# bigmat18/cuda-mesh-voxelization

Measured on AMD Instinct MI355X. Metric: Mvoxels/s (voxelize+JFA) at N=512, bunny 1.35M tris, higher is better.
Workload: dtype f32

## Files before the change

cuda_mesh_voxelization_amd/csrc/jfa_dense.hip:

```cpp
#include "jfa_common.h"

namespace vp {
namespace {

template <class ID> constexpr bool final_mask_global() { return ID::kTab > 512; }
constexpr int kStoreAux = 2;
template <int PM>
__device__ __forceinline__ float from_partner(float v)
{
    constexpr int ctrl = PM == 1 ? 0xB1 : PM == 2 ? 0x4E : PM == 4 ? 0x141 : 0x128;
    return __builtin_bit_cast(float, __builtin_amdgcn_update_dpp(0, __builtin_bit_cast(int, v), ctrl, 0xf, 0xf, true));
}
template <class ID, int RY, int NT, bool FINAL>
constexpr int dense_waves()
{
    return std::is_same<ID, IdC>::value ? 4 : RY > 4 ? 4 : (FINAL && !final_mask_global<ID>()) ? (ID::kTab == 512 ? 5 : 4) : (ID::kTab == 512 || NT == 512) ? 6 : 4;
}
template <class ID, int RY, int CH, int NT, bool FINAL, int PM, int CLOSED = 0, bool FULL = false, bool CYC = false>
__global__ void __launch_bounds__(NT, (dense_waves<ID, RY, NT, FINAL>()))
jfa_pass_dense(Frame f, uint32_t kArg, uint32_t ka, const char* __restrict__ in, const char* __restrict__ inB, char* __restrict__ out, char* __restrict__ outB,
               const char* __restrict__ none_row, const uint32_t* __restrict__ words, float fill, float* __restrict__ sdf,
               uint32_t tilesY, uint32_t tiles, uint32_t splitTiles, uint32_t cyc)
{
    static_assert(!CYC || !FINAL, "the last pass (k = 1) is never a multiple of the rank count");
    using T = typename ID::T;
    constexpr bool CPT = std::is_same<ID, IdC>::value;
    constexpr uint32_t IDB = 4u;
    constexpr int TAB = ID::kTab;
    constexpr int PXT = CPT ? TAB : TAB + 1;
    constexpr int TABZ = CPT ? IdC::kTabZ : TAB;
    constexpr int HY = (CLOSED & 1) ? 0 : 1;
    constexpr bool CZ = (CLOSED & 2) != 0;
    constexpr int NR = RY + 2 * HY;
    static_assert(!CLOSED || !FINAL, "closed tiles: id passes");
    constexpr int NC = PM ? 2 : 3;
    constexpr int NI = NR * NC;
    constexpr int CHT = CPT ? 1 : CH;
    using B = typename std::conditional<FINAL, float, double>::type;
    __shared__ float PX[PXT];
    __shared__ float TY[RY][TAB];
    __shared__ float TZ[CHT][TABZ];
    __shared__ uint32_t RB[CPT ? (CH + 2) * NR : 1];
    constexpr bool GM = final_mask_global<ID>();
    __shared__ uint32_t WM[(FINAL && !GM) ? RY * CH * (TAB / 32) : 1];

    const int N = (int)f.n;
    const uint32_t k = FINAL ? 1u : kArg;
    const int K = (int)k;
    const int zsh = CYC ? (int)(cyc & 31u) : 0, zoff = CYC ? (int)(cyc >> 8) : 0;
    const int KZ = CYC ? K >> zsh : K, NZ = CYC ? N >> zsh : N;
    auto zglobal = [&](int l) { return CYC ? zoff + (l << zsh) : l; };
    const int nzl = (int)(f.z1 - f.z0);
    const uint32_t tid = threadIdx.x;
    const int nresY = min(K, N);
    const bool rev = ((31 - __builtin_clz(k)) & 1) != 0;
    uint32_t lin = blockIdx.x;
    const uint32_t total = tiles;
    uint32_t xpart = 0, xparts = 1;
    if (lin >= total - splitTiles) {
        const uint32_t u = lin - (total - splitTiles);
        lin = total - splitTiles + (u >> 1); xpart = u & 1u; xparts = 2;
    }
    {
        const uint32_t whole8 = (total - splitTiles) & ~7u;
        if (K < 8 && lin < whole8) lin = (lin & 7u) * (whole8 >> 3) + (lin >> 3);
    }
    if (rev) lin = total - 1u - lin;
    const int nres = min(KZ, nzl);
    uint32_t bx, by, bxq, bxr, byq, byr;
    udivmod(lin, tilesY, by, bx); udivmod(bx, (uint32_t)nresY, bxq, bxr);
    const int ybase = (int)bxr + (int)bxq * RY * K;
    udivmod(by, (uint32_t)nres, byq, byr);
    const int lbase = (int)byr + (int)byq * CH * KZ;
    if (ybase >= N || lbase >= nzl) return;
    const int zbase = lbase + (int)f.z0;
    const int KA = (int)ka;
    float py[RY], pz[CH];
#pragma unroll
    for (int j = 0; j < RY; ++j) py[j] = axis_pos(f.oy, ybase + j * K, f.vs);
#pragma unroll
    for (int j = 0; j < CH; ++j) pz[j] = axis_pos(f.oz, zglobal(zbase + j * KZ), f.vs);
    for (uint32_t i = tid; i < (uint32_t)PXT; i += NT) PX[i] = i < (uint32_t)N ? axis_pos(f.ox, i, f.vs) : INFINITY;
    for (uint32_t i = tid; i < (uint32_t)TAB; i += NT) {
        if (i < (uint32_t)N) {
            const uint32_t si = scr(i);
            const float sy = axis_pos(f.oy, i, f.vs), sz = axis_pos(f.oz, i, f.vs);
#pragma unroll
            for (int j = 0; j < RY; ++j) { const float d = sy - py[j]; TY[j][si] = d * d; }
            if (CPT) TZ[0][si] = sz;
            else {
#pragma unroll
                for (int j = 0; j < CHT; ++j) { const float d = sz - pz[j]; TZ[j][si] = d * d; }
            }
        } else {
#pragma unroll
            for (int j = 0; j < RY; ++j) TY[j][i] = 0.0f;
#pragma unroll
            for (int j = 0; j < CHT; ++j) TZ[j][i] = 0.0f;
        }
    }
    if constexpr (TABZ > TAB)
        for (uint32_t i = (uint32_t)TAB + tid; i < (uint32_t)TABZ; i += NT) TZ[0][i] = INFINITY;
    if (CPT) {
        for (uint32_t i = tid; i < (uint32_t)((CH + 2) * NR); i += NT) {
            const int pj = (int)(i / NR) - 1, zg = zbase + pj * KZ, yy = ybase + ((int)(i % NR) - HY) * K;
            const bool ok = zg >= (int)f.z0 - KZ && zg < (int)f.z1 + KZ && zg >= 0 && zg < NZ && yy >= 0 && yy < N;
            RB[i] = ok ? (uint32_t)((lbase + pj * KA) * N + yy) : 0u;
        }
    }
    if (FINAL && !GM) {
        for (uint32_t i = tid; i < (uint32_t)(RY * CH) * f.w; i += NT) {
            uint32_t ou, c;
            udivmod(i, f.w, ou, c);
            const int o = (int)ou, a = o / CH, j = o % CH;
            const int oy = ybase + a * K, oz = zbase + j * K;
            WM[o * (TAB / 32) + (int)c] = (oy < N && oz < (int)f.z1) ? words[(uint32_t)((oz - (int)f.z0) * N + oy) * f.w + c] : 0u;
        }
    }
    __syncthreads();

    const char* tx = reinterpret_cast<const char*>(PX);
    const char* ty = reinterpret_cast<const char*>(TY);
    const char* tz = reinterpret_cast<const char*>(TZ);
    const uint32_t rowBytes = (uint32_t)N * IDB;
    const size_t planeBytes = (size_t)N * rowBytes;
    const char* noneB = none_row + (size_t)TAB * 4u;
    int yout = 1, nout = 1;
    if constexpr (FULL) { yout = RY; nout = CH; }
    else {
#pragma unroll
        for (int j = 1; j < RY; ++j) yout += (ybase + j * K < N) ? 1 : 0;
#pragma unroll
        for (int j = 1; j < CH; ++j) nout += (zbase + j * KZ < (int)f.z1) ? 1 : 0;
    }
    const uint32_t kb = k * IDB;

    const int zbase0 = zbase, lbase0 = lbase, ybase0 = ybase;
    const uint32_t xiters = ((uint32_t)N + NT - 1) / NT, xper = (xiters + xparts - 1) / xparts * NT;
    const uint32_t xbeg = xpart * xper, xend = min((uint32_t)N, xbeg + xper);
    for (uint32_t xb = xbeg; xb < xend; xb += NT) {
        uint32_t x = xb + tid;
        bool upper = false;
        if constexpr (PM != 0) {
            uint32_t pl;
            if (PM == 1) { upper = tid & 1u; pl = tid >> 1; }
            else if (PM == 2) { upper = (tid >> 1) & 1u; pl = ((tid >> 2) << 1) | (tid & 1u); }
            else if (PM == 4) { const uint32_t l8 = tid & 7u; upper = l8 >> 2; pl = ((tid >> 3) << 2) | (upper ? 7u - l8 : l8); }
            else { upper = (tid >> 3) & 1u; pl = ((tid >> 4) << 3) | (tid & 7u); }
            const uint32_t pr = (xb >> 1) + pl;
            x = (((pr & ~(k - 1u)) << 1) | (pr & (k - 1u))) + (upper ? k : 0u);
        } else if (x >= xend) break;
        const int zbase = (int)opaque_uniform((size_t)(uint32_t)zbase0), lbase = (int)opaque_uniform((size_t)(uint32_t)lbase0);
        const int ybase = (int)opaque_uniform((size_t)(uint32_t)ybase0);
        const int plo = zbase - KZ >= 0 ? -1 : 0;
        const char* gbase = in + (ptrdiff_t)(lbase + plo * KA) * (ptrdiff_t)planeBytes;
        uint32_t ro[NR];
        bool yv[NR];
#pragma unroll
        for (int rr = 0; rr < NR; ++rr) {
            const int ny = ybase + (rr - HY) * K;
            yv[rr] = ny >= 0 && ny < N && max(rr - HY - 1, 0) < yout;
            ro[rr] = (uint32_t)(yv[rr] ? ny : 0) * rowBytes;
        }
        const float px = PX[x];
        const bool hasM = x >= k, hasP = x + k < (uint32_t)N;
        const uint32_t xo = x * IDB, xmo = hasM ? xo - kb : xo, xpo = hasP ? xo + kb : xo;
        const uint32_t xpart = upper ? xo - kb : xo + kb, xout = upper ? xpo : xmo;
        const uint32_t xoB = xo >> 2, xmoB = xmo >> 2, xpoB = xpo >> 2, xoutB = xout >> 2;

        struct Plane { const char* base; const char* baseB; bool ok; };
        auto plane_of = [&](int P, bool needed) {
            Plane pl;
            const int zg = zbase + P * KZ;
            pl.ok = needed && zg >= 0 && zg < NZ;
            const ptrdiff_t wp = pl.ok ? (ptrdiff_t)(lbase + P * KA) : 0;
            pl.base = opaque_uniform(in + wp * (ptrdiff_t)planeBytes);
            pl.baseB = CPT ? opaque_uniform(inB + wp * (ptrdiff_t)((size_t)N * N)) : nullptr;
            return pl;
        };
        auto load_row = [&](const Plane& pl, int rr, T (&w)[NI]) {
            const bool ok = pl.ok && yv[rr];
            const __amdgpu_buffer_rsrc_t b = row_resource(ok ? pl.base + ro[rr] : none_row, rowBytes);
            if constexpr (CPT) {
                const __amdgpu_buffer_rsrc_t bb = row_resource(ok ? pl.baseB + (ro[rr] >> 2) : noneB, (uint32_t)N);
                if constexpr (PM != 0) {
                    uint32_t w0, w1;
                    row_load(w0, b, xo); row_load(w1, b, xout);
                    w[rr * 2 + 0] = make_uint2(w0, row_load_u8(bb, xoB));
                    w[rr * 2 + 1] = make_uint2(w1, row_load_u8(bb, xoutB));
                } else {
                    uint32_t w0, w1, w2;
                    row_load(w0, b, xmo); row_load(w1, b, xo); row_load(w2, b, xpo);
                    w[rr * 3 + 0] = make_uint2(w0, row_load_u8(bb, xmoB));
                    w[rr * 3 + 1] = make_uint2(w1, row_load_u8(bb, xoB));
                    w[rr * 3 + 2] = make_uint2(w2, row_load_u8(bb, xpoB));
                }
            } else if constexpr (PM != 0) {
                row_load(w[rr * 2 + 0], b, xo);
                row_load(w[rr * 2 + 1], b, xout);
            } else {
                row_load(w[rr * 3 + 0], b, xmo);
                row_load(w[rr * 3 + 1], b, xo);
                row_load(w[rr * 3 + 2], b, xpo);
            }
        };

        B best[RY][CH];

        struct Dec { float sx; float dy2[RY]; float dz2[CH]; uint32_t zt; };
        auto lookup = [&](int P, int rr, T id, Dec& d) {
            const int alo = max(rr - HY - 1, 0), ahi = min(rr - HY + 1, RY - 1), olo = max(P - 1, 0), ohi = min(P + 1, CH - 1);
            d.sx = lds_f32(tx + ID::xoff(id));
            if constexpr (CPT) d.zt = ID::zt2(id); else d.zt = 0u;
            const uint32_t yo = ID::yoff(id), zo = ID::zoff(id);
#pragma unroll
            for (int a = alo; a <= ahi; ++a) d.dy2[a] = lds_f32(ty + a * (TAB * 4) + yo);
            if constexpr (CPT) {
                const float sz = lds_f32(tz + zo);
#pragma unroll
                for (int o = olo; o <= ohi; ++o) { const float dzv = sz - pz[o]; d.dz2[o] = dzv * dzv; }
            } else {
#pragma unroll
                for (int o = olo; o <= ohi; ++o) d.dz2[o] = lds_f32(tz + o * (TAB * 4) + zo);
            }
        };
        float hold[3][3];
        auto steps_col = [&](int P, int rr, int c, bool ownCol, uint32_t coloff, const Dec& d, uint32_t prank, auto dppv) {
            constexpr bool DPPV = decltype(dppv)::value;
            auto val = [&](float v) { if constexpr (DPPV) return from_partner<PM ? PM : 1>(v); else return v; };
            auto valu = [&](uint32_t v) { if constexpr (DPPV) return __float_as_uint(from_partner<PM ? PM : 1>(__uint_as_float(v))); else return v; };
            const int alo = max(rr - HY - 1, 0), ahi = min(rr - HY + 1, RY - 1), olo = max(P - 1, 0), ohi = min(P + 1, CH - 1);
            const float dxv = val(d.sx) - px;
            const float dx2 = dxv * dxv;
            u32x2 cand;
            if (!FINAL) {
                if constexpr (CPT) cand.x = (uint32_t)(((P + 1) * NR + rr + 1) << 14) + 1u + coloff + valu(d.zt);
                else cand.x = prank + ro[rr] + coloff;
            }
#pragma unroll
            for (int a = alo; a <= ahi; ++a) {
                const float pre = val(d.dy2[a]) + dx2;
                const bool ownRow = (rr == a + HY) && ownCol;
#pragma unroll
                for (int o = olo; o <= ohi; ++o) {
                    const float dd = val(d.dz2[o]) + pre;
                    if constexpr (FINAL) {
                        if (c == 0) hold[a - alo][o - olo] = dd;
                        else if (c == 1) best[a][o] = min3_f32(best[a][o], hold[a - alo][o - olo], dd);
                        else best[a][o] = min_f32(best[a][o], dd);
                    } else {
                        u32x2 cd = cand;
                        if (ownRow && o == P) cd.x = CPT ? d.zt : 0u;
                        cd.y = __float_as_uint(dd);
                        best[a][o] = min_f64(best[a][o], __builtin_bit_cast(double, cd));
                    }
                }
            }
        };
        auto steps = [&](int P, int rr, int c, const Dec& d, uint32_t prank) {
            if constexpr (PM != 0) {
                if (c == 0) {
                    steps_col(P, rr, 0, true, xo, d, prank, std::false_type{});
                    steps_col(P, rr, 1, false, xpart, d, prank, std::true_type{});
                } else {
                    steps_col(P, rr, 2, false, xout, d, prank, std::false_type{});
                }
            } else {
                steps_col(P, rr, c, c == 1, c == 0 ? xmo : c == 1 ? xo : xpo, d, prank, std::false_type{});
            }
        };
        constexpr bool PIPE = ID::kTab == 512 || (FINAL && !CPT);
        auto scatter = [&](int P, T (&w)[NI]) {
            const uint32_t prank = CPT ? 0u : (uint32_t)((P - plo) * KA) * (uint32_t)planeBytes + 1u;
            const int olo = max(P - 1, 0), ohi = min(P + 1, CH - 1);
            Plane next{nullptr, nullptr, false};
            const bool roll = P + 1 <= CH - (CZ ? 1 : 0);
            if (roll) next = plane_of(P + 1, P + 1 <= nout);
            if constexpr (PIPE) {
                constexpr int DEPTH = (FINAL && ID::kTab == 1024) ? 2 : 1;
                Dec d[DEPTH + 1];
#pragma unroll
                for (int j = 0; j < DEPTH && j < NI; ++j) lookup(P, j / NC, w[j], d[j]);
#pragma unroll
                for (int j = 0; j < NI; ++j) {
                    const int rr = j / NC, c = j % NC;
                    if (j + DEPTH < NI) lookup(P, (j + DEPTH) / NC, w[j + DEPTH], d[(j + DEPTH) % (DEPTH + 1)]);
                    __builtin_amdgcn_sched_barrier(0);
                    steps(P, rr, c, d[j % (DEPTH + 1)], prank);
                    if (c == NC - 1) {
                        const int alo = max(rr - HY - 1, 0), ahi = min(rr - HY + 1, RY - 1);
#pragma unroll
                        for (int a = alo; a <= ahi; ++a)
#pragma unroll
                            for (int o = olo; o <= ohi; ++o) pin(best[a][o]);
                        if (roll) load_row(next, rr, w);
                    }
                    __builtin_amdgcn_sched_barrier(0);
                }
                return;
            }
#pragma unroll
            for (int rr = 0; rr < NR; ++rr) {
                const int alo = max(rr - HY - 1, 0), ahi = min(rr - HY + 1, RY - 1);
#pragma unroll
                for (int c = 0; c < NC; ++c) {
                    Dec d;
                    lookup(P, rr, w[rr * NC + c], d);
                    steps(P, rr, c, d, prank);
                }
#pragma unroll
                for (int a = alo; a <= ahi; ++a)
#pragma unroll
                    for (int o = olo; o <= ohi; ++o) pin(best[a][o]);
                if (roll) load_row(next, rr, w);
            }
        };

        T w[NI];
        T pend[RY];
        {
            const Plane first = plane_of(CZ ? 0 : -1, true);
#pragma unroll
            for (int rr = 0; rr < NR; ++rr) load_row(first, rr, w);
        }
#pragma clang loop unroll(full)
        for (int P = -1; P <= CH; ++P) {
            if (P + 1 < CH) {
#pragma unroll
                for (int a = 0; a < RY; ++a) {
                    if constexpr (FINAL) best[a][P + 1] = INFINITY;
                    else best[a][P + 1] = __builtin_bit_cast(double, (u32x2){0xFFFFFFFFu, 0x7F800000u});
                }
            }
            uint32_t mw[RY] = {};
            if constexpr (FINAL && GM) {
                if (P >= 1 && P - 1 < nout) {
                    const char* wpl = opaque_uniform(reinterpret_cast<const char*>(words) + ((size_t)(lbase + (P - 1) * K) * N + ybase) * (size_t)(f.w * 4u));
                    const __amdgpu_buffer_rsrc_t wr = row_resource(wpl, (uint32_t)(RY * K) * f.w * 4u);
#pragma unroll
                    for (int a = 0; a < RY; ++a) {
                        if (a >= yout) continue;
                        mw[a] = (uint32_t)__builtin_amdgcn_raw_buffer_load_b32(wr, (int)((x >> 5) << 2), (int)((uint32_t)(a * K) * f.w * 4u), 0);
                    }
                }
            }
            if (!(CZ && (P == -1 || P == CH))) scatter(P, w);
            if constexpr (FINAL) {
                if (P >= 1 && P - 1 < nout) {
                    const char* spl = opaque_uniform(reinterpret_cast<const char*>(sdf) + ((size_t)(lbase + (P - 1) * K) * N + ybase) * (size_t)rowBytes);
                    const __amdgpu_buffer_rsrc_t sr = row_resource(spl, (uint32_t)((RY - 1) * K + 1) * rowBytes);
#pragma unroll
                    for (int a = 0; a < RY; ++a) {
                        if (a >= yout) continue;
                        const bool set = ((GM ? mw[a] : WM[(a * CH + (P - 1)) * (TAB / 32) + (x >> 5)]) >> (x & 31)) & 1u;
                        __builtin_amdgcn_raw_buffer_store_b32(__float_as_uint(set ? best[a][P - 1] : copysignf(best[a][P - 1], fill)), sr, (int)xo,
                                                              (int)((uint32_t)(a * K) * rowBytes), kStoreAux);
                    }
                }
            } else {
                if (P >= 2 && P - 2 < nout) {
                    const char* orow = opaque_uniform(out + ((size_t)(lbase + (P - 2) * KA) * N + ybase) * rowBytes);
                    const char* orowB = CPT ? opaque_uniform(outB + ((size_t)(lbase + (P - 2) * KA) * N + ybase) * (size_t)N) : nullptr;
#pragma unroll
                    for (int a = 0; a < RY; ++a) {
                        if (a >= yout) continue;
                        if constexpr (CPT) {
                            row_store<kStoreAux>(pend[a].x, row_resource(orow + (size_t)(a * K) * rowBytes, rowBytes), xo);
                            row_store_u8<kStoreAux>(pend[a].y, row_resource(orowB + (size_t)(a * K) * N, (uint32_t)N), xoB);
                        } else {
                            row_store<kStoreAux>(pend[a], row_resource(orow + (size_t)(a * K) * rowBytes, rowBytes), xo);
                        }
                    }
                }
                if (P >= 1 && P - 1 < nout) {
                    const uint32_t orank = (uint32_t)((P - 1 - plo) * KA) * (uint32_t)planeBytes;
#pragma unroll
                    for (int a = 0; a < RY; ++a) {
                        if (a >= yout) continue;
                        const uint32_t lo = __builtin_bit_cast(u32x2, best[a][P - 1]).x;
                        if constexpr (CPT) {
                            const uint32_t zt = lo & 2u;
                            const uint32_t r = lo < 4u ? (uint32_t)((P * NR + a + HY + 1) << 14) + xo : lo - 1u - zt;
                            const ptrdiff_t row = (ptrdiff_t)(int)RB[(r >> 14) - 1u];
                            const uint32_t none1 = __builtin_bit_cast(u32x2, best[a][P - 1]).y == 0x7F800000u ? IdC::kNoneBit : 0u;
                            pend[a] = make_uint2(*reinterpret_cast<const uint32_t*>(in + row * (ptrdiff_t)rowBytes + (ptrdiff_t)(r & 16383u)),
                                                 zt | none1);
                        } else {
                            const uint32_t ownOff = orank + ro[a + HY] + xo;
                            const uint32_t off = lo ? lo - 1u : ownOff;
                            pend[a] = *reinterpret_cast<const T*>(gbase + off);
                        }
                    }
                }
            }
#pragma unroll
            for (int a = 0; a < RY; ++a)
#pragma unroll
                for (int o = P; o <= P + 1; ++o)
                    if (o >= 0 && o < CH) pin(best[a][o]);
        }
        if constexpr (!FINAL) {
            if (CH - 1 < nout) {
                const char* orow = opaque_uniform(out + ((size_t)(lbase + (CH - 1) * KA) * N + ybase) * rowBytes);
                const char* orowB = CPT ? opaque_uniform(outB + ((size_t)(lbase + (CH - 1) * KA) * N + ybase) * (size_t)N) : nullptr;
#pragma unroll
                for (int a = 0; a < RY; ++a) {
                    if (a >= yout) continue;
                    if constexpr (CPT) {
                        row_store<kStoreAux>(pend[a].x, row_resource(orow + (size_t)(a * K) * rowBytes, rowBytes), xo);
                        row_store_u8<kStoreAux>(pend[a].y, row_resource(orowB + (size_t)(a * K) * N, (uint32_t)N), xoB);
                    } else {
                        row_store<kStoreAux>(pend[a], row_resource(orow + (size_t)(a * K) * rowBytes, rowBytes), xo);
                    }
                }
            }
        }
    }
}

}

static uint32_t tail_split(const vp_ctx* ctx, uint32_t tiles, uint32_t wgPerCu)
{
    const uint32_t slots = (uint32_t)ctx->cus * wgPerCu;
    if (tiles >= 16u * slots) return 0;
    return std::min(tiles / 2u, slots * 4u / 3u);
}

struct DenseArgs {
    vp_ctx* ctx; Frame f; uint32_t k, ka;
    const char *in, *inB; char *out, *outB; const char* none_row;
    const uint32_t* words; float fill; float* sdf;
    uint32_t nresY, ylen, nres, zlen;
    uint32_t cyc = 0;
};
int launch_dense_id9_tile16(const DenseArgs& a, bool pairsOk);

namespace {

template <class ID, int RY, int CH, int NT, bool F, int PM, int CL = 0, bool FULL = false, bool CYC = false>
void launch_tile(const DenseArgs& a)
{
    const uint32_t ty = a.nresY * ((a.ylen + RY - 1) / RY), t = ty * a.nres * ((a.zlen + CH - 1) / CH);
    constexpr uint32_t perCu = std::is_same<ID, IdC>::value ? 2u
                             : ID::kTab == 512 ? (RY == 8 ? 4u : (F && !final_mask_global<ID>()) ? 5u : 6u)
                             : NT == 512 ? (RY == 8 ? 2u : 3u) : 4u;
    const uint32_t sp = a.f.n > (uint32_t)NT ? tail_split(a.ctx, t, perCu) : 0u;
    hipLaunchKernelGGL((jfa_pass_dense<ID, RY, CH, NT, F, PM, CL, FULL, CYC>), dim3(t + sp), dim3(NT), 0, a.ctx->stream, a.f, a.k, a.ka,
                       a.in, a.inB, a.out, a.outB, a.none_row, a.words, a.fill, a.sdf, ty, t, sp, a.cyc);
}

template <int V> using int_c = std::integral_constant<int, V>;

template <class ID, int CH, int NT, bool F, bool ALWAYS_FULL = false, bool CYC = false>
void launch_shape(const DenseArgs& a, bool pairsOk, bool wholeChains)
{
    constexpr int RY = (ID::kTab == 512 && !F && CH >= 8) ? 8 : 4;
    constexpr bool canFull = CH >= 8 && (ID::kTab != 1024 || F);
    auto go = [&](auto pm) {
        constexpr int PM = decltype(pm)::value;
        if constexpr (ALWAYS_FULL || (CYC && canFull)) launch_tile<ID, RY, CH, NT, F, PM, 0, true, CYC>(a);
        else {
            if constexpr (canFull) {
                if (wholeChains && a.ylen % RY == 0) { launch_tile<ID, RY, CH, NT, F, PM, 0, true>(a); return; }
            }
            launch_tile<ID, RY, CH, NT, F, PM, 0, false, CYC>(a);
        }
    };
    if constexpr (CH >= 8) {
        if (pairsOk && a.f.n % NT == 0) {
            if constexpr (F) { go(int_c<1>{}); return; }
            else {
                if constexpr (ID::kTab != 512) { if (a.k == 2) { go(int_c<2>{}); return; } }
                if (a.k == 4) { go(int_c<4>{}); return; }
                if (a.k >= 8) { go(int_c<8>{}); return; }
            }
        }
    }
    go(int_c<0>{});
}

template <class ID, bool FIN>
int launch_dense(vp_ctx* ctx, const Frame& f, uint32_t k, const IdWin& in, const IdWin& out, uint32_t stride,
                 const uint32_t* d_words, float fill, float* d_sdf)
{
    const uint32_t nz = f.z1 - f.z0, n = f.n;
    constexpr bool fin = FIN;
    const uint32_t nres = std::min(k, nz), zlen = (nz + k - 1) / k;
    const uint32_t nresY = std::min(k, n), ylen = (n + k - 1) / k;
    if (stride == k && nz % k == 0 && k < nz && zlen > 8 && zlen % 8 != 0) {
        const uint32_t planesA = (zlen / 8u) * 8u * k;
        Frame fa = f, fb = f;
        fa.z1 = f.z0 + planesA; fb.z0 = fa.z1;
        IdWin inB = in, outB = out;
        inB.at += planesA; outB.at += planesA;
        const size_t wordPlane = (size_t)n * f.w, sdfPlane = (size_t)n * n;
        VP_TRY((launch_dense<ID, FIN>(ctx, fa, k, in, out, stride, d_words, fill, d_sdf)));
        return launch_dense<ID, FIN>(ctx, fb, k, inB, outB, stride, d_words ? d_words + planesA * wordPlane : nullptr, fill, d_sdf ? d_sdf + planesA * sdfPlane : nullptr);
    }
    if (FIN && k != 1) return set_error(VP_ERR_INVALID, "jfa_pass_dense: the fused last pass is the pass with k = 1");
    VP_TRY(ensure_none_rows(ctx));
    DenseArgs a{ctx, f, k, stride, win_words(in, n, in.at), win_compact(n) ? win_bytes_plane(in, n, in.at) : nullptr,
                win_words(out, n, out.at), win_compact(n) ? win_bytes_plane(out, n, out.at) : nullptr,
                (const char*)(std::is_same<ID, Id9>::value ? none_row_id9(ctx) : std::is_same<ID, Id10>::value ? none_row_id10(ctx) : none_row_idc(ctx)),
                d_words, fill, d_sdf, nresY, ylen, nres, zlen};
    const bool pow2 = (n & (n - 1)) == 0;
    const bool wholeChains = zlen % 8 == 0 && nz % k == 0 && n % k == 0;
    constexpr int NTD = ID::kTab == 512 ? 256 : 512;
    constexpr int NTS = ID::kTab == 2048 ? 512 : 256;
    if constexpr (!std::is_same<ID, IdC>::value) {
        if constexpr (!fin) {
            if (pow2 && stride == k && f.z0 == 0 && f.z1 == n && n == 8u * k && n % NTD == 0) {
                launch_tile<ID, 8, 8, NTD, false, 8, 3, ID::kTab == 512>(a);
                VP_HIP(hipGetLastError());
                return 0;
            }
        }
    }
    const bool deep = zlen % 8 == 0 || (zlen > 4 && zlen < 8);
    const bool tiny = zlen <= 2;
    if constexpr (std::is_same<ID, IdC>::value) {
        if (zlen % 16 == 0 && stride == k) {
            launch_shape<ID, 16, NTD, fin>(a, pow2 && (fin || k >= 2), wholeChains);
            VP_HIP(hipGetLastError());
            return 0;
        }
    }
    if constexpr (ID::kTab == 512) {
        if (n == 512 && zlen % 16 == 0 && stride == k && wholeChains) {
            if constexpr (fin) launch_shape<ID, 16, 512, true, true>(a, pow2, true);
            else VP_TRY(launch_dense_id9_tile16(a, pow2 && k >= 2));
            VP_HIP(hipGetLastError());
            return 0;
        }
    }
    if (deep) launch_shape<ID, 8, NTD, fin>(a, pow2 && (fin || k >= 2), wholeChains);
    else if constexpr (!fin) { if (tiny) launch_shape<ID, 2, NTS, false>(a, false, false); else launch_shape<ID, 4, NTS, false>(a, false, false); }
    else launch_shape<ID, 4, NTS, true>(a, false, false);
    VP_HIP(hipGetLastError());
    return 0;
}

template <class ID>
int launch_dense_cyclic(vp_ctx* ctx, const Frame& f, uint32_t k, const IdWin& in, const IdWin& out, uint32_t ranks, uint32_t rank)
{
    const uint32_t n = f.n, zsh = (uint32_t)__builtin_ctz(ranks);
    const uint32_t nzl = n >> zsh, kz = k >> zsh;
    if ((ranks & (ranks - 1)) != 0 || rank >= ranks || n % ranks != 0 || k % ranks != 0 || n % k != 0 || n / k < 8 || ((n / k) & (n / k - 1)) != 0)
        return set_error(VP_ERR_INVALID, "jfa_pass_dense (cyclic): n = %u, k = %u, %u ranks", n, k, ranks);
    VP_TRY(ensure_none_rows(ctx));
    Frame fl = f;
    fl.z0 = 0; fl.z1 = nzl;
    const uint32_t zlen = nzl / kz, ylen = n / k;
    DenseArgs a{ctx, fl, k, kz, win_words(in, n, in.at), win_compact(n) ? win_bytes_plane(in, n, in.at) : nullptr,
                win_words(out, n, out.at), win_compact(n) ? win_bytes_plane(out, n, out.at) : nullptr,
                (const char*)(std::is_same<ID, Id9>::value ? none_row_id9(ctx) : std::is_same<ID, Id10>::value ? none_row_id10(ctx) : none_row_idc(ctx)),
                nullptr, 0.0f, nullptr, std::min(k, n), ylen, std::min(kz, nzl), zlen, zsh | (rank << 8)};
    const bool pow2 = (n & (n - 1)) == 0;
    constexpr int NTD = ID::kTab == 512 ? 256 : 512;
    if constexpr (!std::is_same<ID, IdC>::value) {
        if (pow2 && n == 8u * k && n % NTD == 0) {
            launch_tile<ID, 8, 8, NTD, false, 8, 3, ID::kTab == 512, true>(a);
            VP_HIP(hipGetLastError());
            return 0;
        }
    }
    if constexpr (std::is_same<ID, IdC>::value) {
        if (zlen % 16 == 0) {
            launch_shape<ID, 16, NTD, false, false, true>(a, pow2 && k >= 2, true);
            VP_HIP(hipGetLastError());
            return 0;
        }
    }
    launch_shape<ID, 8, NTD, false, false, true>(a, pow2 && k >= 2, true);
    VP_HIP(hipGetLastError());
    return 0;
}

}

#ifndef VP_DENSE_PART
#define VP_DENSE_PART 0
#endif
#define VP_DENSE_ENTRY(PART, NAME, ID, FIN)                                                                                                \
    int NAME(vp_ctx* ctx, const Frame& f, uint32_t k, const IdWin& in, const IdWin& out, uint32_t stride, const uint32_t* d_words, float fill, float* d_sdf) \
    { return launch_dense<ID, FIN>(ctx, f, k, in, out, stride, d_words, fill, d_sdf); }
#if VP_DENSE_PART == 0 || VP_DENSE_PART == 1
VP_DENSE_ENTRY(1, launch_dense_id9_pass, Id9, false)
#endif
#if VP_DENSE_PART == 0 || VP_DENSE_PART == 2
VP_DENSE_ENTRY(2, launch_dense_id9_last, Id9, true)
#endif
#if VP_DENSE_PART == 0 || VP_DENSE_PART == 3
VP_DENSE_ENTRY(3, launch_dense_id10_pass, Id10, false)
#endif
#if VP_DENSE_PART == 0 || VP_DENSE_PART == 4
VP_DENSE_ENTRY(4, launch_dense_id10_last, Id10, true)
#endif
#if VP_DENSE_PART == 0 || VP_DENSE_PART == 5
VP_DENSE_ENTRY(5, launch_dense_idc_pass, IdC, false)
#endif
#if VP_DENSE_PART == 0 || VP_DENSE_PART == 6
VP_DENSE_ENTRY(6, launch_dense_idc_last, IdC, true)
#endif
#if VP_DENSE_PART == 0 || VP_DENSE_PART == 7
int launch_dense_id9_tile16(const DenseArgs& a, bool pairsOk) { launch_shape<Id9, 16, 512, false, true>(a, pairsOk, true); return 0; }
#endif
#undef VP_DENSE_ENTRY
#define VP_CYCLIC_ENTRY(NAME, ID)                                                                                                        \
    int NAME(vp_ctx* ctx, const Frame& f, uint32_t k, const IdWin& in, const IdWin& out, uint32_t ranks, uint32_t rank)                 \
    { return launch_dense_cyclic<ID>(ctx, f, k, in, out, ranks, rank); }
#if VP_DENSE_PART == 0 || VP_DENSE_PART == 8
VP_CYCLIC_ENTRY(launch_cyclic_id9_pass, Id9)
#endif
#if VP_DENSE_PART == 0 || VP_DENSE_PART == 9
VP_CYCLIC_ENTRY(launch_cyclic_id10_pass, Id10)
#endif
#if VP_DENSE_PART == 0 || VP_DENSE_PART == 10
VP_CYCLIC_ENTRY(launch_cyclic_idc_pass, IdC)
#endif
#undef VP_CYCLIC_ENTRY

}
```

Measured before the change: 49430.

## Add chain-end tile variants that skip absent halo rows and planes in JFA passes

Splits the dense JFA pass body into a device function and adds ENDS-specialised launches for k=32 and k=16 at N=512. Tiles at the ends of a y or z chain are walked in mirrored direction, so the missing neighbour row or plane is always on the low side and can be dropped at compile time. The closed-tile flags are split into separate lo/hi bits. This cuts halo loads and distance evaluations for edge tiles, at the cost of more template instances, run-time branching between variants and negative-stride addressing.

```diff
diff --git a/cuda_mesh_voxelization_amd/csrc/jfa_dense.hip b/cuda_mesh_voxelization_amd/csrc/jfa_dense.hip
--- a/cuda_mesh_voxelization_amd/csrc/jfa_dense.hip
+++ b/cuda_mesh_voxelization_amd/csrc/jfa_dense.hip
@@ -11,38 +11,52 @@
     constexpr int ctrl = PM == 1 ? 0xB1 : PM == 2 ? 0x4E : PM == 4 ? 0x141 : 0x128;
     return __builtin_bit_cast(float, __builtin_amdgcn_update_dpp(0, __builtin_bit_cast(int, v), ctrl, 0xf, 0xf, true));
 }
+constexpr int kNoRowLo = 1, kNoRowHi = 2;
+constexpr int kNoPlaneLo = 4, kNoPlaneHi = 8;
+constexpr int kClosedTile = kNoRowLo | kNoRowHi | kNoPlaneLo | kNoPlaneHi;
 template <class ID, int RY, int NT, bool FINAL>
 constexpr int dense_waves()
 {
     return std::is_same<ID, IdC>::value ? 4 : RY > 4 ? 4 : (FINAL && !final_mask_global<ID>()) ? (ID::kTab == 512 ? 5 : 4) : (ID::kTab == 512 || NT == 512) ? 6 : 4;
 }
-template <class ID, int RY, int CH, int NT, bool FINAL, int PM, int CLOSED = 0, bool FULL = false, bool CYC = false>
-__global__ void __launch_bounds__(NT, (dense_waves<ID, RY, NT, FINAL>()))
-jfa_pass_dense(Frame f, uint32_t kArg, uint32_t ka, const char* __restrict__ in, const char* __restrict__ inB, char* __restrict__ out, char* __restrict__ outB,
-               const char* __restrict__ none_row, const uint32_t* __restrict__ words, float fill, float* __restrict__ sdf,
-               uint32_t tilesY, uint32_t tiles, uint32_t splitTiles, uint32_t cyc)
-{
-    static_assert(!CYC || !FINAL, "the last pass (k = 1) is never a multiple of the rank count");
+
+template <class ID, int RY, int CH, bool FINAL>
+struct DenseLds {
+    static constexpr bool CPT = std::is_same<ID, IdC>::value;
+    static constexpr int TAB = ID::kTab;
+    static constexpr int PXT = CPT ? TAB : TAB + 1;
+    static constexpr int TABZ = CPT ? IdC::kTabZ : TAB;
+    static constexpr int CHT = CPT ? 1 : CH;
+    static constexpr int RBN = CPT ? (CH + 2) * (RY + 2) : 1;
+    static constexpr int WMN = (FINAL && !final_mask_global<ID>()) ? RY * CH * (TAB / 32) : 1;
+    float (&PX)[PXT];
+    float (&TY)[RY][TAB];
+    float (&TZ)[CHT][TABZ];
+    uint32_t (&RB)[RBN];
+    uint32_t (&WM)[WMN];
+};
+
+template <class ID, int RY, int CH, int NT, bool FINAL, int PM, int CLOSED, bool FULL, bool CYC, bool MIR = false>
+__device__ __forceinline__ void
+dense_tile(const DenseLds<ID, RY, CH, FINAL>& lds, const Frame& f, uint32_t kArg, uint32_t ka, const char* __restrict__ in, const char* __restrict__ inB,
+           char* __restrict__ out, char* __restrict__ outB, const char* __restrict__ none_row, const uint32_t* __restrict__ words, float fill,
+           float* __restrict__ sdf, uint32_t cyc, uint32_t xpart, uint32_t xparts, int ybase, int lbase, bool miry, bool mirz)
+{
     using T = typename ID::T;
-    constexpr bool CPT = std::is_same<ID, IdC>::value;
+    using LDS = DenseLds<ID, RY, CH, FINAL>;
+    constexpr bool CPT = LDS::CPT;
     constexpr uint32_t IDB = 4u;
-    constexpr int TAB = ID::kTab;
-    constexpr int PXT = CPT ? TAB : TAB + 1;
-    constexpr int TABZ = CPT ? IdC::kTabZ : TAB;
-    constexpr int HY = (CLOSED & 1) ? 0 : 1;
-    constexpr bool CZ = (CLOSED & 2) != 0;
-    constexpr int NR = RY + 2 * HY;
-    static_assert(!CLOSED || !FINAL, "closed tiles: id passes");
+    constexpr int TAB = LDS::TAB, PXT = LDS::PXT, TABZ = LDS::TABZ, CHT = LDS::CHT;
+    constexpr int HYlo = (CLOSED & kNoRowLo) ? 0 : 1, HYhi = (CLOSED & kNoRowHi) ? 0 : 1;
+    constexpr bool NZlo = (CLOSED & kNoPlaneLo) != 0, NZhi = (CLOSED & kNoPlaneHi) != 0;
+    constexpr int NR = RY + HYlo + HYhi;
+    static_assert(!CLOSED || (!FINAL && !CPT), "closed tiles: id passes on 32-bit ids");
+    static_assert(!MIR || (!FINAL && !CPT && !CYC && FULL), "run-time walk directions: whole tiles of the 32-bit id passes");
     constexpr int NC = PM ? 2 : 3;
     constexpr int NI = NR * NC;
-    constexpr int CHT = CPT ? 1 : CH;
     using B = typename std::conditional<FINAL, float, double>::type;
-    __shared__ float PX[PXT];
-    __shared__ float TY[RY][TAB];
-    __shared__ float TZ[CHT][TABZ];
-    __shared__ uint32_t RB[CPT ? (CH + 2) * NR : 1];
+    auto& PX = lds.PX; auto& TY = lds.TY; auto& TZ = lds.TZ; auto& RB = lds.RB; auto& WM = lds.WM;
     constexpr bool GM = final_mask_global<ID>();
-    __shared__ uint32_t WM[(FINAL && !GM) ? RY * CH * (TAB / 32) : 1];
 
     const int N = (int)f.n;
     const uint32_t k = FINAL ? 1u : kArg;
@@ -50,36 +64,15 @@
     const int zsh = CYC ? (int)(cyc & 31u) : 0, zoff = CYC ? (int)(cyc >> 8) : 0;
     const int KZ = CYC ? K >> zsh : K, NZ = CYC ? N >> zsh : N;
     auto zglobal = [&](int l) { return CYC ? zoff + (l << zsh) : l; };
-    const int nzl = (int)(f.z1 - f.z0);
     const uint32_t tid = threadIdx.x;
-    const int nresY = min(K, N);
-    const bool rev = ((31 - __builtin_clz(k)) & 1) != 0;
-    uint32_t lin = blockIdx.x;
-    const uint32_t total = tiles;
-    uint32_t xpart = 0, xparts = 1;
-    if (lin >= total - splitTiles) {
-        const uint32_t u = lin - (total - splitTiles);
-        lin = total - splitTiles + (u >> 1); xpart = u & 1u; xparts = 2;
-    }
-    {
-        const uint32_t whole8 = (total - splitTiles) & ~7u;
-        if (K < 8 && lin < whole8) lin = (lin & 7u) * (whole8 >> 3) + (lin >> 3);
-    }
-    if (rev) lin = total - 1u - lin;
-    const int nres = min(KZ, nzl);
-    uint32_t bx, by, bxq, bxr, byq, byr;
-    udivmod(lin, tilesY, by, bx); udivmod(bx, (uint32_t)nresY, bxq, bxr);
-    const int ybase = (int)bxr + (int)bxq * RY * K;
-    udivmod(by, (uint32_t)nres, byq, byr);
-    const int lbase = (int)byr + (int)byq * CH * KZ;
-    if (ybase >= N || lbase >= nzl) return;
     const int zbase = lbase + (int)f.z0;
     const int KA = (int)ka;
+    const int SK = (MIR && miry) ? -K : K, SKZ = (MIR && mirz) ? -KZ : KZ, SKA = (MIR && mirz) ? -KA : KA;
     float py[RY], pz[CH];
 #pragma unroll
-    for (int j = 0; j < RY; ++j) py[j] = axis_pos(f.oy, ybase + j * K, f.vs);
-#pragma unroll
-    for (int j = 0; j < CH; ++j) pz[j] = axis_pos(f.oz, zglobal(zbase + j * KZ), f.vs);
+    for (int j = 0; j < RY; ++j) py[j] = axis_pos(f.oy, ybase + j * SK, f.vs);
+#pragma unroll
+    for (int j = 0; j < CH; ++j) pz[j] = axis_pos(f.oz, zglobal(zbase + j * SKZ), f.vs);
     for (uint32_t i = tid; i < (uint32_t)PXT; i += NT) PX[i] = i < (uint32_t)N ? axis_pos(f.ox, i, f.vs) : INFINITY;
     for (uint32_t i = tid; i < (uint32_t)TAB; i += NT) {
         if (i < (uint32_t)N) {
@@ -103,7 +96,7 @@
         for (uint32_t i = (uint32_t)TAB + tid; i < (uint32_t)TABZ; i += NT) TZ[0][i] = INFINITY;
     if (CPT) {
         for (uint32_t i = tid; i < (uint32_t)((CH + 2) * NR); i += NT) {
-            const int pj = (int)(i / NR) - 1, zg = zbase + pj * KZ, yy = ybase + ((int)(i % NR) - HY) * K;
+            const int pj = (int)(i / NR) - 1, zg = zbase + pj * KZ, yy = ybase + ((int)(i % NR) - HYlo) * K;
             const bool ok = zg >= (int)f.z0 - KZ && zg < (int)f.z1 + KZ && zg >= 0 && zg < NZ && yy >= 0 && yy < N;
             RB[i] = ok ? (uint32_t)((lbase + pj * KA) * N + yy) : 0u;
         }
@@ -152,14 +145,14 @@
         } else if (x >= xend) break;
         const int zbase = (int)opaque_uniform((size_t)(uint32_t)zbase0), lbase = (int)opaque_uniform((size_t)(uint32_t)lbase0);
         const int ybase = (int)opaque_uniform((size_t)(uint32_t)ybase0);
-        const int plo = zbase - KZ >= 0 ? -1 : 0;
-        const char* gbase = in + (ptrdiff_t)(lbase + plo * KA) * (ptrdiff_t)planeBytes;
+        const int plo = (MIR && mirz) ? ((!NZhi && zbase + CH * SKZ >= 0) ? CH : CH - 1) : ((!NZlo && zbase - KZ >= 0) ? -1 : 0);
+        const char* gbase = in + (ptrdiff_t)(lbase + plo * SKA) * (ptrdiff_t)planeBytes;
         uint32_t ro[NR];
         bool yv[NR];
 #pragma unroll
         for (int rr = 0; rr < NR; ++rr) {
-            const int ny = ybase + (rr - HY) * K;
-            yv[rr] = ny >= 0 && ny < N && max(rr - HY - 1, 0) < yout;
+            const int ny = ybase + (rr - HYlo) * SK;
+            yv[rr] = ny >= 0 && ny < N && max(rr - HYlo - 1, 0) < yout;
             ro[rr] = (uint32_t)(yv[rr] ? ny : 0) * rowBytes;
         }
         const float px = PX[x];
@@ -171,9 +164,9 @@
         struct Plane { const char* base; const char* baseB; bool ok; };
         auto plane_of = [&](int P, bool needed) {
             Plane pl;
-            const int zg = zbase + P * KZ;
+            const int zg = zbase + P * SKZ;
             pl.ok = needed && zg >= 0 && zg < NZ;
-            const ptrdiff_t wp = pl.ok ? (ptrdiff_t)(lbase + P * KA) : 0;
+            const ptrdiff_t wp = pl.ok ? (ptrdiff_t)(lbase + P * SKA) : 0;
             pl.base = opaque_uniform(in + wp * (ptrdiff_t)planeBytes);
             pl.baseB = CPT ? opaque_uniform(inB + wp * (ptrdiff_t)((size_t)N * N)) : nullptr;
             return pl;
@@ -209,7 +202,7 @@
 
         struct Dec { float sx; float dy2[RY]; float dz2[CH]; uint32_t zt; };
         auto lookup = [&](int P, int rr, T id, Dec& d) {
-            const int alo = max(rr - HY - 1, 0), ahi = min(rr - HY + 1, RY - 1), olo = max(P - 1, 0), ohi = min(P + 1, CH - 1);
+            const int alo = max(rr - HYlo - 1, 0), ahi = min(rr - HYlo + 1, RY - 1), olo = max(P - 1, 0), ohi = min(P + 1, CH - 1);
             d.sx = lds_f32(tx + ID::xoff(id));
             if constexpr (CPT) d.zt = ID::zt2(id); else d.zt = 0u;
             const uint32_t yo = ID::yoff(id), zo = ID::zoff(id);
@@ -229,7 +222,7 @@
             constexpr bool DPPV = decltype(dppv)::value;
             auto val = [&](float v) { if constexpr (DPPV) return from_partner<PM ? PM : 1>(v); else return v; };
             auto valu = [&](uint32_t v) { if constexpr (DPPV) return __float_as_uint(from_partner<PM ? PM : 1>(__uint_as_float(v))); else return v; };
-            const int alo = max(rr - HY - 1, 0), ahi = min(rr - HY + 1, RY - 1), olo = max(P - 1, 0), ohi = min(P + 1, CH - 1);
+            const int alo = max(rr - HYlo - 1, 0), ahi = min(rr - HYlo + 1, RY - 1), olo = max(P - 1, 0), ohi = min(P + 1, CH - 1);
             const float dxv = val(d.sx) - px;
             const float dx2 = dxv * dxv;
             u32x2 cand;
@@ -240,7 +233,7 @@
 #pragma unroll
             for (int a = alo; a <= ahi; ++a) {
                 const float pre = val(d.dy2[a]) + dx2;
-                const bool ownRow = (rr == a + HY) && ownCol;
+                const bool ownRow = (rr == a + HYlo) && ownCol;
 #pragma unroll
                 for (int o = olo; o <= ohi; ++o) {
                     const float dd = val(d.dz2[o]) + pre;
@@ -271,10 +264,10 @@
         };
         constexpr bool PIPE = ID::kTab == 512 || (FINAL && !CPT);
         auto scatter = [&](int P, T (&w)[NI]) {
-            const uint32_t prank = CPT ? 0u : (uint32_t)((P - plo) * KA) * (uint32_t)planeBytes + 1u;
+            const uint32_t prank = CPT ? 0u : (uint32_t)((P - plo) * SKA) * (uint32_t)planeBytes + 1u;
             const int olo = max(P - 1, 0), ohi = min(P + 1, CH - 1);
             Plane next{nullptr, nullptr, false};
-            const bool roll = P + 1 <= CH - (CZ ? 1 : 0);
+            const bool roll = P + 1 <= CH - (NZhi ? 1 : 0);
             if (roll) next = plane_of(P + 1, P + 1 <= nout);
             if constexpr (PIPE) {
                 constexpr int DEPTH = (FINAL && ID::kTab == 1024) ? 2 : 1;
@@ -288,7 +281,7 @@
                     __builtin_amdgcn_sched_barrier(0);
                     steps(P, rr, c, d[j % (DEPTH + 1)], prank);
                     if (c == NC - 1) {
-                        const int alo = max(rr - HY - 1, 0), ahi = min(rr - HY + 1, RY - 1);
+                        const int alo = max(rr - HYlo - 1, 0), ahi = min(rr - HYlo + 1, RY - 1);
 #pragma unroll
                         for (int a = alo; a <= ahi; ++a)
 #pragma unroll
@@ -301,7 +294,7 @@
             }
 #pragma unroll
             for (int rr = 0; rr < NR; ++rr) {
-                const int alo = max(rr - HY - 1, 0), ahi = min(rr - HY + 1, RY - 1);
+                const int alo = max(rr - HYlo - 1, 0), ahi = min(rr - HYlo + 1, RY - 1);
 #pragma unroll
                 for (int c = 0; c < NC; ++c) {
                     Dec d;
@@ -319,7 +312,7 @@
         T w[NI];
         T pend[RY];
         {
-            const Plane first = plane_of(CZ ? 0 : -1, true);
+            const Plane first = plane_of(NZlo ? 0 : -1, true);
 #pragma unroll
             for (int rr = 0; rr < NR; ++rr) load_row(first, rr, w);
         }
@@ -344,7 +337,7 @@
                     }
                 }
             }
-            if (!(CZ && (P == -1 || P == CH))) scatter(P, w);
+            if (!((NZlo && P == -1) || (NZhi && P == CH))) scatter(P, w);
             if constexpr (FINAL) {
                 if (P >= 1 && P - 1 < nout) {
                     const char* spl = opaque_uniform(reinterpret_cast<const char*>(sdf) + ((size_t)(lbase + (P - 1) * K) * N + ybase) * (size_t)rowBytes);
@@ -359,8 +352,8 @@
                 }
             } else {
                 if (P >= 2 && P - 2 < nout) {
-                    const char* orow = opaque_uniform(out + ((size_t)(lbase + (P - 2) * KA) * N + ybase) * rowBytes);
-                    const char* orowB = CPT ? opaque_uniform(outB + ((size_t)(lbase + (P - 2) * KA) * N + ybase) * (size_t)N) : nullptr;
+                    const char* orow = opaque_uniform(out + ((size_t)(lbase + (P - 2) * SKA) * N + ybase) * rowBytes);
+                    const char* orowB = CPT ? opaque_uniform(outB + ((size_t)(lbase + (P - 2) * SKA) * N + ybase) * (size_t)N) : nullptr;
 #pragma unroll
                     for (int a = 0; a < RY; ++a) {
                         if (a >= yout) continue;
@@ -368,25 +361,26 @@
                             row_store<kStoreAux>(pend[a].x, row_resource(orow + (size_t)(a * K) * rowBytes, rowBytes), xo);
                             row_store_u8<kStoreAux>(pend[a].y, row_resource(orowB + (size_t)(a * K) * N, (uint32_t)N), xoB);
                         } else {
-                            row_store<kStoreAux>(pend[a], row_resource(orow + (size_t)(a * K) * rowBytes, rowBytes), xo);
+                            if constexpr (MIR) row_store<kStoreAux>(pend[a], row_resource(orow + (ptrdiff_t)(a * SK) * (ptrdiff_t)rowBytes, rowBytes), xo);
+                            else row_store<kStoreAux>(pend[a], row_resource(orow + (size_t)(a * K) * rowBytes, rowBytes), xo);
                         }
                     }
                 }
                 if (P >= 1 && P - 1 < nout) {
-                    const uint32_t orank = (uint32_t)((P - 1 - plo) * KA) * (uint32_t)planeBytes;
+                    const uint32_t orank = (uint32_t)((P - 1 - plo) * SKA) * (uint32_t)planeBytes;
 #pragma unroll
                     for (int a = 0; a < RY; ++a) {
                         if (a >= yout) continue;
                         const uint32_t lo = __builtin_bit_cast(u32x2, best[a][P - 1]).x;
                         if constexpr (CPT) {
                             const uint32_t zt = lo & 2u;
-                            const uint32_t r = lo < 4u ? (uint32_t)((P * NR + a + HY + 1) << 14) + xo : lo - 1u - zt;
+                            const uint32_t r = lo < 4u ? (uint32_t)((P * NR + a + HYlo + 1) << 14) + xo : lo - 1u - zt;
                             const ptrdiff_t row = (ptrdiff_t)(int)RB[(r >> 14) - 1u];
                             const uint32_t none1 = __builtin_bit_cast(u32x2, best[a][P - 1]).y == 0x7F800000u ? IdC::kNoneBit : 0u;
                             pend[a] = make_uint2(*reinterpret_cast<const uint32_t*>(in + row * (ptrdiff_t)rowBytes + (ptrdiff_t)(r & 16383u)),
                                                  zt | none1);
                         } else {
-                            const uint32_t ownOff = orank + ro[a + HY] + xo;
+                            const uint32_t ownOff = orank + ro[a + HYlo] + xo;
                             const uint32_t off = lo ? lo - 1u : ownOff;
                             pend[a] = *reinterpret_cast<const T*>(gbase + off);
                         }
@@ -401,8 +395,8 @@
         }
         if constexpr (!FINAL) {
             if (CH - 1 < nout) {
-                const char* orow = opaque_uniform(out + ((size_t)(lbase + (CH - 1) * KA) * N + ybase) * rowBytes);
-                const char* orowB = CPT ? opaque_uniform(outB + ((size_t)(lbase + (CH - 1) * KA) * N + ybase) * (size_t)N) : nullptr;
+                const char* orow = opaque_uniform(out + ((size_t)(lbase + (CH - 1) * SKA) * N + ybase) * rowBytes);
+                const char* orowB = CPT ? opaque_uniform(outB + ((size_t)(lbase + (CH - 1) * SKA) * N + ybase) * (size_t)N) : nullptr;
 #pragma unroll
                 for (int a = 0; a < RY; ++a) {
                     if (a >= yout) continue;
@@ -410,10 +404,75 @@
                         row_store<kStoreAux>(pend[a].x, row_resource(orow + (size_t)(a * K) * rowBytes, rowBytes), xo);
                         row_store_u8<kStoreAux>(pend[a].y, row_resource(orowB + (size_t)(a * K) * N, (uint32_t)N), xoB);
                     } else {
-                        row_store<kStoreAux>(pend[a], row_resource(orow + (size_t)(a * K) * rowBytes, rowBytes), xo);
+                        if constexpr (MIR) row_store<kStoreAux>(pend[a], row_resource(orow + (ptrdiff_t)(a * SK) * (ptrdiff_t)rowBytes, rowBytes), xo);
+                        else row_store<kStoreAux>(pend[a], row_resource(orow + (size_t)(a * K) * rowBytes, rowBytes), xo);
                     }
                 }
             }
+        }
+    }
+}
+
+template <class ID, int RY, int CH, int NT, bool FINAL, int PM, int CLOSED = 0, bool FULL = false, bool CYC = false, int ENDS = 0>
+__global__ void __launch_bounds__(NT, (dense_waves<ID, RY, NT, FINAL>()))
+jfa_pass_dense(Frame f, uint32_t kArg, uint32_t ka, const char* __restrict__ in, const char* __restrict__ inB, char* __restrict__ out, char* __restrict__ outB,
+               const char* __restrict__ none_row, const uint32_t* __restrict__ words, float fill, float* __restrict__ sdf,
+               uint32_t tilesY, uint32_t tiles, uint32_t splitTiles, uint32_t cyc)
+{
+    static_assert(!CYC || !FINAL, "the last pass (k = 1) is never a multiple of the rank count");
+    static_assert(!ENDS || (!CLOSED && FULL && !CYC && !FINAL), "chain-end tiles: whole tiles of the id passes of a whole grid");
+    using LDS = DenseLds<ID, RY, CH, FINAL>;
+    __shared__ float PX[LDS::PXT];
+    __shared__ float TY[RY][LDS::TAB];
+    __shared__ float TZ[LDS::CHT][LDS::TABZ];
+    __shared__ uint32_t RB[LDS::RBN];
+    __shared__ uint32_t WM[LDS::WMN];
+    const LDS lds{PX, TY, TZ, RB, WM};
+
+    const int N = (int)f.n;
+    const uint32_t k = FINAL ? 1u : kArg;
+    const int K = (int)k;
+    const int KZ = CYC ? K >> (int)(cyc & 31u) : K;
+    const int nzl = (int)(f.z1 - f.z0);
+    const int nresY = min(K, N);
+    const bool rev = ((31 - __builtin_clz(k)) & 1) != 0;
+    uint32_t lin = blockIdx.x;
+    const uint32_t total = tiles;
+    uint32_t xpart = 0, xparts = 1;
+    if (lin >= total - splitTiles) {
+        const uint32_t u = lin - (total - splitTiles);
+        lin = total - splitTiles + (u >> 1); xpart = u & 1u; xparts = 2;
+    }
+    {
+        const uint32_t whole8 = (total - splitTiles) & ~7u;
+        if (K < 8 && lin < whole8) lin = (lin & 7u) * (whole8 >> 3) + (lin >> 3);
+    }
+    if (rev) lin = total - 1u - lin;
+    const int nres = min(KZ, nzl);
+    uint32_t bx, by, bxq, bxr, byq, byr;
+    udivmod(lin, tilesY, by, bx); udivmod(bx, (uint32_t)nresY, bxq, bxr);
+    const int ybase = (int)bxr + (int)bxq * RY * K;
+    udivmod(by, (uint32_t)nres, byq, byr);
+    const int lbase = (int)byr + (int)byq * CH * KZ;
+    if (ybase >= N || lbase >= nzl) return;
+    auto tile = [&](auto closed, auto mir, int y0, int l0, bool miry, bool mirz) {
+        dense_tile<ID, RY, CH, NT, FINAL, PM, decltype(closed)::value, FULL, CYC, decltype(mir)::value>(
+            lds, f, kArg, ka, in, inB, out, outB, none_row, words, fill, sdf, cyc, xpart, xparts, y0, l0, miry, mirz);
+    };
+    using std::integral_constant;
+    if constexpr (ENDS == 0) tile(integral_constant<int, CLOSED>{}, std::false_type{}, ybase, lbase, false, false);
+    else {
+        constexpr uint32_t rowTiles = 1u << ENDS, plTiles = rowTiles / 2u;
+        const bool miry = bxq == rowTiles - 1u, mirz = plTiles > 1u && byq == plTiles - 1u;
+        const bool rowEnd = bxq == 0u || miry, plEnd = byq == 0u || mirz;
+        const int y0 = miry ? ybase + (RY - 1) * K : ybase, l0 = mirz ? lbase + (CH - 1) * KZ : lbase;
+        if constexpr (plTiles == 1u)
+            tile(integral_constant<int, kNoRowLo | kNoPlaneLo | kNoPlaneHi>{}, std::true_type{}, y0, l0, miry, false);
+        else if (rowEnd && plEnd) tile(integral_constant<int, kNoRowLo | kNoPlaneLo>{}, std::true_type{}, y0, l0, miry, mirz);
+        else if (plEnd) tile(integral_constant<int, kNoPlaneLo>{}, std::true_type{}, y0, l0, false, mirz);
+        else if constexpr (plTiles > 2u) {
+            if (rowEnd) tile(integral_constant<int, kNoRowLo>{}, std::true_type{}, y0, l0, miry, false);
+            else tile(integral_constant<int, 0>{}, std::false_type{}, ybase, lbase, false, false);
         }
     }
 }
@@ -438,7 +497,7 @@
 
 namespace {
 
-template <class ID, int RY, int CH, int NT, bool F, int PM, int CL = 0, bool FULL = false, bool CYC = false>
+template <class ID, int RY, int CH, int NT, bool F, int PM, int CL = 0, bool FULL = false, bool CYC = false, int ENDS = 0>
 void launch_tile(const DenseArgs& a)
 {
     const uint32_t ty = a.nresY * ((a.ylen + RY - 1) / RY), t = ty * a.nres * ((a.zlen + CH - 1) / CH);
@@ -446,7 +505,7 @@
                              : ID::kTab == 512 ? (RY == 8 ? 4u : (F && !final_mask_global<ID>()) ? 5u : 6u)
                              : NT == 512 ? (RY == 8 ? 2u : 3u) : 4u;
     const uint32_t sp = a.f.n > (uint32_t)NT ? tail_split(a.ctx, t, perCu) : 0u;
-    hipLaunchKernelGGL((jfa_pass_dense<ID, RY, CH, NT, F, PM, CL, FULL, CYC>), dim3(t + sp), dim3(NT), 0, a.ctx->stream, a.f, a.k, a.ka,
+    hipLaunchKernelGGL((jfa_pass_dense<ID, RY, CH, NT, F, PM, CL, FULL, CYC, ENDS>), dim3(t + sp), dim3(NT), 0, a.ctx->stream, a.f, a.k, a.ka,
                        a.in, a.inB, a.out, a.outB, a.none_row, a.words, a.fill, a.sdf, ty, t, sp, a.cyc);
 }
 
@@ -511,7 +570,7 @@
     if constexpr (!std::is_same<ID, IdC>::value) {
         if constexpr (!fin) {
             if (pow2 && stride == k && f.z0 == 0 && f.z1 == n && n == 8u * k && n % NTD == 0) {
-                launch_tile<ID, 8, 8, NTD, false, 8, 3, ID::kTab == 512>(a);
+                launch_tile<ID, 8, 8, NTD, false, 8, kClosedTile, ID::kTab == 512>(a);
                 VP_HIP(hipGetLastError());
                 return 0;
             }
@@ -560,7 +619,7 @@
     constexpr int NTD = ID::kTab == 512 ? 256 : 512;
     if constexpr (!std::is_same<ID, IdC>::value) {
         if (pow2 && n == 8u * k && n % NTD == 0) {
-            launch_tile<ID, 8, 8, NTD, false, 8, 3, ID::kTab == 512, true>(a);
+            launch_tile<ID, 8, 8, NTD, false, 8, kClosedTile, ID::kTab == 512, true>(a);
             VP_HIP(hipGetLastError());
             return 0;
         }
@@ -604,7 +663,14 @@
 VP_DENSE_ENTRY(6, launch_dense_idc_last, IdC, true)
 #endif
 #if VP_DENSE_PART == 0 || VP_DENSE_PART == 7
-int launch_dense_id9_tile16(const DenseArgs& a, bool pairsOk) { launch_shape<Id9, 16, 512, false, true>(a, pairsOk, true); return 0; }
+int launch_dense_id9_tile16(const DenseArgs& a, bool pairsOk)
+{
+    const bool whole = a.f.z0 == 0 && a.f.z1 == a.f.n && a.ka == a.k && a.f.n == 512;
+    if (pairsOk && whole && a.k == 32) launch_tile<Id9, 8, 16, 512, false, 8, 0, true, false, 1>(a);
+    else if (pairsOk && whole && a.k == 16) launch_tile<Id9, 8, 16, 512, false, 8, 0, true, false, 2>(a);
+    else launch_shape<Id9, 16, 512, false, true>(a, pairsOk, true);
+    return 0;
+}
 #endif
 #undef VP_DENSE_ENTRY
 #define VP_CYCLIC_ENTRY(NAME, ID)                                                                                                        \
```

New measurement: 49800, median of 6. No clear change (+0.8%).
